# rishikksh20/FastSpeech2

Hardware: NVIDIA H100
Metric: mel-frames/sec (batched inference) (higher is better)
Workload: dtype 3xf16

## Files before the change

fastspeech2_b200/csrc/gemm_tc.cu:

```cuda
#include <stdlib.h>

#include "tc_common.cuh"

namespace fs2 {
namespace {
using namespace tc;

constexpr int BM = 128;
constexpr int BK = 32;
constexpr int A_BYTES = BM * BK * 4;
constexpr int THREADS = 384;
constexpr int RING_BUDGET = 227 * 1024 - 1024  - 256 ;

struct TcParams {
  int L, tiles_per_utt;
  int m_tiles, n_tiles;
  int B, full, gn, upt, full_tiles;
  int K, taps, pad;
  const float* bias; const float* resid; int ldr; int act;
  float* out; int ldo;
  float a_inv; const float* w_inv;
  __half* outp; __half* outp_lo; int ldo_p;
  float* vt_out; __half* vtp; __half* vtp_lo; int vt_col0, vt_dk, vt_heads, vt_lpad, vt_L;
  const int64_t* lens;
};

template <int BN, bool PRECISE, bool HALF = false>
struct Cfg {
  static constexpr int B_BYTES = BN * BK * 4;
  static constexpr int STAGE_BYTES = (PRECISE ? 2 : 1) * (A_BYTES + B_BYTES);
  static_assert(!PRECISE || HALF, "the error-compensated family is 3xF16");
  static constexpr int STAGES = (RING_BUDGET / STAGE_BYTES) > 8 ? 8 : (RING_BUDGET / STAGE_BYTES);
  static constexpr size_t SMEM = (size_t)STAGES * STAGE_BYTES + 1024 + 256;
  static constexpr int BKE = HALF ? 2 * BK : BK;
  static constexpr int A_LO = A_BYTES;
  static constexpr int B_HI = PRECISE ? 2 * A_BYTES : A_BYTES;
  static constexpr int B_LO = B_HI + B_BYTES;
  static constexpr uint32_t TX_BYTES = (PRECISE ? 2 : 1) * (A_BYTES + B_BYTES);
  static_assert(BN % 16 == 0 && BN >= 16 && BN <= 128, "tile width: sums of wgmma N = 128 / 64 / 16");
  static_assert(B_BYTES % 1024 == 0, "B stage must keep 1024-byte alignment");
  static_assert(STAGES >= 2, "resources");
};

template <int BN, bool HALF, int C0 = 0>
__device__ __forceinline__ void mma_tile(float* d, uint64_t a, uint64_t b, uint32_t acc) {
  if constexpr (BN - C0 >= 128) {
    if constexpr (HALF) wgmma_f16_n128(d + C0 / 2, a, b + (C0 * 128 >> 4), acc); else wgmma_tf32_n128(d + C0 / 2, a, b + (C0 * 128 >> 4), acc);
    mma_tile<BN, HALF, C0 + 128>(d, a, b, acc);
  } else if constexpr (BN - C0 >= 64) {
    if constexpr (HALF) wgmma_f16_n64(d + C0 / 2, a, b + (C0 * 128 >> 4), acc); else wgmma_tf32_n64(d + C0 / 2, a, b + (C0 * 128 >> 4), acc);
    mma_tile<BN, HALF, C0 + 64>(d, a, b, acc);
  } else if constexpr (BN - C0 >= 16) {
    if constexpr (HALF) wgmma_f16_n16(d + C0 / 2, a, b + (C0 * 128 >> 4), acc); else wgmma_tf32_n16(d + C0 / 2, a, b + (C0 * 128 >> 4), acc);
    mma_tile<BN, HALF, C0 + 16>(d, a, b, acc);
  }
}

template <int BN, bool PRECISE, bool HALF>
__global__ void __launch_bounds__(THREADS, 1)
tap_gemm_tc_kernel(const __grid_constant__ CUtensorMap tmap_a, const __grid_constant__ CUtensorMap tmap_b,
                   const __grid_constant__ CUtensorMap tmap_b_lo, const __grid_constant__ CUtensorMap tmap_a16, TcParams p) {
  using C = Cfg<BN, PRECISE, HALF>;
  extern __shared__ uint8_t smem_raw[];
  uint8_t* tiles = smem_raw + ((1024u - (smem_u32(smem_raw) & 1023u)) & 1023u);
  uint64_t* full_bar = reinterpret_cast<uint64_t*>(tiles + (size_t)C::STAGES * C::STAGE_BYTES);
  uint64_t* empty_bar = full_bar + C::STAGES;

  const int warp = uniform_warp_idx(), lane = threadIdx.x & 31;
  const int kchunks = (p.K + C::BKE - 1) / C::BKE;
  const int steps = p.taps * kchunks;
  const int total_tiles = p.m_tiles * p.n_tiles;

  if (threadIdx.x == 0) {
    for (int s = 0; s < C::STAGES; ++s) { mbar_init(&full_bar[s], 1); mbar_init(&empty_bar[s], 8); }
    asm volatile("fence.mbarrier_init.release.cluster;" ::: "memory");
  }
  __syncthreads();
  pdl_wait();

  auto tile_coords = [&](int tile, int& n0, int& b, int& t0, int& packed) -> bool {
    const int mt = tile / p.n_tiles;
    n0 = (tile - mt * p.n_tiles) * BN;
    packed = -1;
    if (p.tiles_per_utt == 0) { b = 0; t0 = mt * BM; }
    else if (mt < p.full_tiles) { b = mt / p.full; t0 = (mt - b * p.full) * BM; }
    else { packed = mt - p.full_tiles; b = packed * p.upt; t0 = p.full * BM; }
    return packed < 0 && p.lens != nullptr && t0 >= p.lens[b];
  };

  if (warp == 0) {
    const uint32_t tiles_addr = smem_u32(tiles), full_addr = smem_u32(full_bar);
    int n = 0;
    for (int tile = blockIdx.x; tile < total_tiles; tile += gridDim.x) {
      int n0, b, t0, packed;
      if (tile_coords(tile, n0, b, t0, packed)) continue;
      int j = 0, kc = 0;
      for (int s = 0; s < steps; ++s, ++n) {
        const int slot = n % C::STAGES, round = n / C::STAGES;
        const int k0 = kc * C::BKE, row = t0 + j - p.pad;
        const uint32_t st = tiles_addr + (uint32_t)slot * C::STAGE_BYTES, fb = full_addr + (uint32_t)slot * 8u;
        pin_before(st, fb, k0, row);
        mbar_wait(&empty_bar[slot], (round & 1) ^ 1);
        mbar_expect_tx_elect(fb, C::TX_BYTES);
        if (packed < 0) {
          tma_load_3d_elect(st, &tmap_a, fb, k0, row, b);
          if (PRECISE) tma_load_3d_elect(st + C::A_LO, &tmap_a, fb, k0, row, b + p.B);
        } else {
          for (int g = 0; g < 8; ++g) {
            const int u = g / p.gn, gi = g - u * p.gn;
            const bool real = u < p.upt && b + u < p.B;
            const int oob = PRECISE ? 2 * p.B : p.B;
            tma_load_3d_elect(st + g * (16 * 128), &tmap_a16, fb, k0, row + gi * 16, real ? b + u : oob);
            if (PRECISE) tma_load_3d_elect(st + C::A_LO + g * (16 * 128), &tmap_a16, fb, k0, row + gi * 16, real ? b + u + p.B : oob);
          }
        }
        tma_load_3d_elect(st + C::B_HI, &tmap_b, fb, k0, n0, j);
        if (PRECISE) tma_load_3d_elect(st + C::B_LO, &tmap_b_lo, fb, k0, n0, j);
        if (++kc == kchunks) { kc = 0; ++j; }
      }
    }
  } else if (warp >= 4) {
    const int cg = (warp >> 2) - 1, wq = warp & 3;
    const int r_lo = 64 * cg + 16 * wq + (lane >> 2);
    const int act = p.act, ldr = p.ldr, ldo = p.ldo;
    const float* __restrict__ resid = p.resid; float* __restrict__ out = p.out;
    const bool has_res = resid != nullptr;
    const float oscale = p.a_inv * (p.w_inv ? __ldg(p.w_inv) : 1.0f);
    float d[BN / 2];
    int n = 0;
    for (int tile = blockIdx.x; tile < total_tiles; tile += gridDim.x) {
      int n0, b, t0, packed;
      const int tile_steps = tile_coords(tile, n0, b, t0, packed) ? 0 : steps;
      long m[2]; bool row_ok[2], row_zero[2];
#pragma unroll
      for (int h = 0; h < 2; ++h) {
        const int row = r_lo + 8 * h;
        int bb = b, t = t0 + row;
        bool ok = t < p.L;
        if (packed >= 0) {
          const int g = row >> 4, u = g / p.gn, gi = g - u * p.gn;
          bb += u;
          t = t0 + gi * 16 + (row & 15);
          ok = u < p.upt && bb < p.B && t < p.L;
        }
        m[h] = (long)bb * p.L + t; row_ok[h] = ok;
        row_zero[h] = ok && p.lens != nullptr && t >= p.lens[bb];
        if (has_res && ok) prefetch_l2(resid + m[h] * ldr + n0);
      }
      int prev = -1;
      for (int s = 0; s < tile_steps; ++s, ++n) {
        const int slot = n % C::STAGES, round = n / C::STAGES;
        const uint32_t base = smem_u32(tiles + (size_t)slot * C::STAGE_BYTES);
        const uint64_t a_hi = make_sw128_kmajor_desc(base + cg * (A_BYTES / 2)), b_hi = make_sw128_kmajor_desc(base + C::B_HI);
        const uint64_t a_lo = make_sw128_kmajor_desc(base + C::A_LO + cg * (A_BYTES / 2)), b_lo = make_sw128_kmajor_desc(base + C::B_LO);
        mbar_wait(&full_bar[slot], round & 1);
        wgmma_fence();
#pragma unroll
        for (int k = 0; k < 4; ++k) {
          if (PRECISE) {
            mma_tile<BN, true>(d, a_lo + 2 * k, b_hi + 2 * k, (s | k) != 0);
            mma_tile<BN, true>(d, a_hi + 2 * k, b_lo + 2 * k, 1);
            mma_tile<BN, true>(d, a_hi + 2 * k, b_hi + 2 * k, 1);
          } else {
            mma_tile<BN, HALF>(d, a_hi + 2 * k, b_hi + 2 * k, (s | k) != 0);
          }
        }
        wgmma_commit();
        wgmma_wait<1>();
        pin_regs<BN / 2>(d);
        if (prev >= 0) { __syncwarp(); if (lane == 0) mbar_arrive(&empty_bar[prev]); }
        prev = slot;
      }
      wgmma_wait<0>();
      pin_regs<BN / 2>(d);
      if (prev >= 0) { __syncwarp(); if (lane == 0) mbar_arrive(&empty_bar[prev]); }
      if (tile_steps == 0) {
#pragma unroll
        for (int i = 0; i < BN / 2; ++i) d[i] = 0.f;
      }

      const bool to_vt = (p.vt_out != nullptr || p.vtp != nullptr) && n0 >= p.vt_col0;
#pragma unroll
      for (int h = 0; h < 2; ++h) {
        if (!row_ok[h] || (to_vt && row_zero[h])) continue;
        const long mm = m[h];
#pragma unroll
        for (int jj = 0; jj < BN / 8; ++jj) {
          const int c = 8 * jj + 2 * (lane & 3), col = n0 + c;
          float v0 = d[4 * jj + 2 * h], v1 = d[4 * jj + 2 * h + 1];
          const float b0 = p.bias ? __ldg(p.bias + col) : 0.f, b1 = p.bias ? __ldg(p.bias + col + 1) : 0.f;
          v0 = fmaf(v0, oscale, b0); v1 = fmaf(v1, oscale, b1);
          if (to_vt) {
            const long ub = mm / p.vt_L; const int ut = (int)(mm - ub * p.vt_L);
            const int rel = col - p.vt_col0, hh = rel / p.vt_dk, d0 = rel - hh * p.vt_dk;
            const long o = ((ub * p.vt_heads + hh) * p.vt_dk + d0) * (long)p.vt_lpad + ut;
            if (p.vt_out != nullptr) {
              p.vt_out[o] = v0; p.vt_out[o + p.vt_lpad] = v1;
            } else {
              uint32_t hi, lo;
              split_pair(v0, v1, hi, lo);
              const __half2 h2 = *reinterpret_cast<const __half2*>(&hi), l2 = *reinterpret_cast<const __half2*>(&lo);
              p.vtp[o] = __low2half(h2); p.vtp[o + p.vt_lpad] = __high2half(h2);
              if (p.vtp_lo != nullptr) { p.vtp_lo[o] = __low2half(l2); p.vtp_lo[o + p.vt_lpad] = __high2half(l2); }
            }
            continue;
          }
          if (act == ACT_RELU) { v0 = fmaxf(v0, 0.f); v1 = fmaxf(v1, 0.f); }
          else if (act == ACT_TANH) { v0 = tanhf(v0); v1 = tanhf(v1); }
          if (has_res) {
            const float2 r = __ldg(reinterpret_cast<const float2*>(resid + mm * ldr + col));
            v0 += r.x; v1 += r.y;
          }
          if (row_zero[h]) { v0 = 0.f; v1 = 0.f; }
          if (HALF && p.outp != nullptr) {
            const long off = mm * p.ldo_p + col;
            if (p.outp_lo != nullptr) {
              uint32_t hi, lo;
              split_pair(v0, v1, hi, lo);
              *reinterpret_cast<uint32_t*>(p.outp + off) = hi;
              *reinterpret_cast<uint32_t*>(p.outp_lo + off) = lo;
            } else {
              *reinterpret_cast<uint32_t*>(p.outp + off) = hi_pair(v0, v1);
            }
          }
          if (out != nullptr) *reinterpret_cast<float2*>(out + mm * ldo + col) = make_float2(v0, v1);
        }
      }
    }
  }
  pdl_trigger();
}

__global__ void split_rows_f16_kernel(const float* __restrict__ x, int ldx, long rows, int K, __half* __restrict__ S) {
  pdl_trigger(); pdl_wait();
  const int kq = K >> 2;
  const long quads = rows * kq;
  __half* __restrict__ lo_plane = S + rows * K;
  for (long i = (long)blockIdx.x * blockDim.x + threadIdx.x; i < quads; i += (long)gridDim.x * blockDim.x) {
    const long r = i / kq;
    const int c = (int)(i - r * kq) * 4;
    const float4 v = *reinterpret_cast<const float4*>(x + r * ldx + c);
    uint2 hv, lv;
    split_pair(v.x, v.y, hv.x, lv.x);
    split_pair(v.z, v.w, hv.y, lv.y);
    *reinterpret_cast<uint2*>(S + r * K + c) = hv;
    *reinterpret_cast<uint2*>(lo_plane + r * K + c) = lv;
  }
}

template <int BN, bool PRECISE, bool HALF = false>
int launch(const TapGemm& g, cudaStream_t st) {
  using C = Cfg<BN, PRECISE, HALF>;
  static unsigned long long configured = 0;
  int rc;
  if ((rc = ensure_smem_attr(tap_gemm_tc_kernel<BN, PRECISE, HALF>, C::SMEM, &configured))) return rc;
  TcParams p;
  p.K = g.K; p.taps = g.taps; p.pad = (g.taps - 1) / 2;
  p.bias = g.bias; p.resid = g.resid; p.ldr = g.ldr; p.act = g.act; p.out = g.out; p.ldo = g.ldo;
  const long rows = (long)g.B * g.L;
  p.a_inv = HALF ? g.a_inv : 1.0f; p.w_inv = HALF ? g.w_inv : nullptr;
  p.outp = HALF ? g.outp : nullptr; p.ldo_p = g.ldo_p;
  p.outp_lo = (HALF && g.outp && g.outp_lo) ? g.outp + rows * g.ldo_p : nullptr;
  p.vt_out = HALF ? nullptr : g.vt_out; p.vtp = HALF ? g.vtp : nullptr;
  p.vtp_lo = (HALF && g.vtp && g.outp_lo) ? g.vtp + (long)g.B * g.vt_heads * g.vt_dk * g.vt_lpad : nullptr;
  p.vt_col0 = g.vt_col0; p.vt_dk = g.vt_dk; p.vt_heads = g.vt_heads; p.vt_lpad = g.vt_lpad; p.vt_L = g.L;
  p.lens = g.lens;
  CUtensorMap ma, mb, mb_lo, ma16;
  const int esz = HALF ? 2 : 4;
  constexpr int planes = HALF && PRECISE ? 2 : 1;
  const void* xa = HALF ? (const void*)g.xp : (const void*)g.x;
  const uint64_t row_bytes = HALF ? (uint64_t)g.K * 2 : (uint64_t)g.ldx * 4;
  if (g.taps == 1 && g.lens == nullptr) {
    const uint64_t M = (uint64_t)g.B * g.L;
    p.L = (int)M; p.tiles_per_utt = 0;
    p.m_tiles = (int)((M + BM - 1) / BM);
    p.B = 1; p.full = 0; p.gn = 1; p.upt = 1; p.full_tiles = 0;
    if ((rc = make_map(&ma, xa, g.K, M, planes, row_bytes, row_bytes * M, BM, HALF))) return rc;
    ma16 = ma;
  } else {
    p.L = g.L; p.tiles_per_utt = (g.L + BM - 1) / BM;
    p.B = g.B; p.full = g.L / BM;
    int tail = g.L % BM;
    p.gn = tail ? (tail + 15) / 16 : 1;
    p.upt = tail ? 8 / p.gn : 1;
    if (tail && p.upt == 1) { p.full += 1; tail = 0; p.gn = 1; }
    p.full_tiles = p.full * g.B;
    p.m_tiles = p.full_tiles + (tail ? (g.B + p.upt - 1) / p.upt : 0);
    if ((rc = make_map(&ma, xa, g.K, g.L, (uint64_t)g.B * planes, row_bytes, row_bytes * g.L, BM, HALF))) return rc;
    if ((rc = make_map(&ma16, xa, g.K, g.L, (uint64_t)g.B * planes, row_bytes, row_bytes * g.L, 16, HALF))) return rc;
  }
  p.n_tiles = g.N / BN;
  const void* w_hi = HALF ? (const void*)g.w_hi : (const void*)g.w;
  if ((rc = make_map(&mb, w_hi, g.K, g.N, g.taps, (uint64_t)g.K * esz, (uint64_t)g.K * esz * g.N, BN, HALF))) return rc;
  if ((rc = make_map(&mb_lo, PRECISE ? (const void*)g.w_lo : w_hi, g.K, g.N, g.taps, (uint64_t)g.K * esz, (uint64_t)g.K * esz * g.N, BN, HALF))) return rc;
  const int total = p.m_tiles * p.n_tiles;
  const int grid = total < sm_count_current() ? total : sm_count_current();
  FS2_CUDA_CHECK(launch_pdl(tap_gemm_tc_kernel<BN, PRECISE, HALF>, dim3(grid), dim3(THREADS), C::SMEM, st, ma, mb, mb_lo, ma16, p));
  FS2_LAUNCH_CHECK();
  return FS2_OK;
}

int tile_width(int N) { return N % 128 == 0 ? 128 : N % 80 == 0 ? 80 : N % 64 == 0 ? 64 : N % 32 == 0 ? 32 : 16; }

template <bool PRECISE, bool HALF>
int launch_any(const TapGemm& g, cudaStream_t st) {
  switch (tile_width(g.N)) {
    case 128: return launch<128, PRECISE, HALF>(g, st);
    case 80: return launch<80, PRECISE, HALF>(g, st);
    case 64: return launch<64, PRECISE, HALF>(g, st);
    case 32: return launch<32, PRECISE, HALF>(g, st);
    default: return launch<16, PRECISE, HALF>(g, st);
  }
}

int check_output(const TapGemm& g, const char* who) {
  FS2_REQUIRE((g.taps & 1) == 1, "%s: taps must be odd", who);
  FS2_REQUIRE(g.N % 16 == 0, "%s: N (%d) must be a multiple of 16", who, g.N);
  FS2_REQUIRE(!g.resid || g.ldr % 4 == 0, "%s: row strides must be 16-byte multiples", who);
  FS2_REQUIRE(!g.out || (g.ldo % 8 == 0 && (reinterpret_cast<uintptr_t>(g.out) & 31) == 0), "%s: output rows must be 32-byte aligned", who);
  return FS2_OK;
}
int check_common(const TapGemm& g, const char* who) {
  FS2_REQUIRE(g.K % 4 == 0, "%s: K (%d) must be a multiple of 4", who, g.K);
  FS2_REQUIRE(g.ldx % 4 == 0, "%s: row strides must be 16-byte multiples", who);
  FS2_REQUIRE((reinterpret_cast<uintptr_t>(g.x) & 15) == 0 && (reinterpret_cast<uintptr_t>(g.w) & 15) == 0 && g.out != nullptr,
              "%s: operands must be 16-byte aligned", who);
  return check_output(g, who);
}

}

int tap_gemm_tf32(const TapGemm& g, cudaStream_t st) {
  int rc = check_common(g, "tap_gemm_tf32");
  if (rc) return rc;
  if ((long)g.B * g.L == 0) return FS2_OK;
  return launch_any<false, false>(g, st);
}

int tap_gemm_planes(const TapGemm& g, cudaStream_t st) {
  const char* who = g.precise ? "tap_gemm_planes(3xF16)" : "tap_gemm_planes(f16)";
  FS2_REQUIRE(g.xp && g.w_hi && (!g.precise || g.w_lo) && (g.out || g.outp || g.vtp), "%s: operand planes / an output missing", who);
  FS2_REQUIRE(g.K % 8 == 0, "%s: K (%d) must be a multiple of 8 (16-byte plane rows)", who, g.K);
  FS2_REQUIRE((reinterpret_cast<uintptr_t>(g.xp) & 15) == 0 && (reinterpret_cast<uintptr_t>(g.w_hi) & 15) == 0, "%s: operands must be 16-byte aligned", who);
  FS2_REQUIRE(!g.outp || (g.ldo_p % 16 == 0 && (reinterpret_cast<uintptr_t>(g.outp) & 31) == 0 && (((long)g.B * g.L * g.ldo_p) % 16) == 0),
              "%s: output plane rows must be 32-byte aligned", who);
  {
    const int bn = tile_width(g.N);
    FS2_REQUIRE(!g.vtp || (g.vt_lpad % 8 == 0 && g.N % bn == 0 && g.vt_col0 % bn == 0 && g.vt_dk % 32 == 0),
                "%s: transposed V planes need a 16-byte row pitch and tile-aligned thirds", who);
  }
  int rc = check_output(g, who);
  if (rc) return rc;
  if ((long)g.B * g.L == 0) return FS2_OK;
  return g.precise ? launch_any<true, true>(g, st) : launch_any<false, true>(g, st);
}

int split_rows(const float* x, int ldx, long rows, int K, __half* planes, cudaStream_t st) {
  if (rows == 0) return FS2_OK;
  FS2_REQUIRE(K % 4 == 0 && ldx % 4 == 0, "split_rows: K and the row stride must be multiples of 4");
  const long quads = rows * (K / 4);
  long blocks = (quads + 255) / 256;
  FS2_CUDA_CHECK(launch_pdl(split_rows_f16_kernel, dim3((unsigned)(blocks > 132 * 16 ? 132 * 16 : blocks)), dim3(256), 0, st, x, ldx, rows, K, planes));
  FS2_LAUNCH_CHECK();
  return FS2_OK;
}

namespace {
__global__ void split_f16_kernel(const float* __restrict__ src, __half* __restrict__ hi, __half* __restrict__ lo, long n,
                                 const float* __restrict__ scale) {
  const float s = scale ? __ldg(scale) : 1.0f;
  for (long i = (long)blockIdx.x * blockDim.x + threadIdx.x; i < n; i += (long)gridDim.x * blockDim.x) {
    const float x = fminf(fmaxf(src[i] * s, -65504.f), 65504.f);
    const __half h = __float2half_rn(x);
    hi[i] = h; lo[i] = __float2half_rn(x - __half2float(h));
  }
}
__global__ void weight_scale_kernel(const float* __restrict__ w, long n, float* __restrict__ scale, float* __restrict__ inv) {
  __shared__ float red[32];
  float m = 0.f;
  for (long i = threadIdx.x; i < n; i += blockDim.x) m = fmaxf(m, fabsf(w[i]));
  m = warp_max(m);
  if ((threadIdx.x & 31) == 0) red[threadIdx.x >> 5] = m;
  __syncthreads();
  if (threadIdx.x < 32) {
    m = threadIdx.x < (blockDim.x >> 5) ? red[threadIdx.x] : 0.f;
    m = warp_max(m);
    if (threadIdx.x == 0) {
      int k = 0;
      if (m > 0.f && isfinite(m)) {
        int e;
        frexpf(m, &e);
        k = 14 - e;
        k = k > 60 ? 60 : (k < -60 ? -60 : k);
      }
      scale[0] = ldexpf(1.0f, k); inv[0] = ldexpf(1.0f, -k);
    }
  }
}
}

namespace {
__global__ void planes_to_rows_kernel(const __half* __restrict__ planes, long n, float* __restrict__ out) {
  for (long i = (long)blockIdx.x * blockDim.x + threadIdx.x; i < n; i += (long)gridDim.x * blockDim.x)
    out[i] = (__half2float(planes[i]) + __half2float(planes[n + i])) * kPlaneInv;
}
}

int planes_to_rows(const __half* planes, long n, float* out, cudaStream_t st) {
  if (n == 0) return FS2_OK;
  long blocks = (n + 255) / 256;
  planes_to_rows_kernel<<<(int)(blocks > 1184 ? 1184 : blocks), 256, 0, st>>>(planes, n, out);
  FS2_LAUNCH_CHECK();
  return FS2_OK;
}

int split_f16(const float* src, __half* hi, __half* lo, long n, const float* scale, cudaStream_t st) {
  if (n == 0) return FS2_OK;
  long blocks = (n + 255) / 256;
  split_f16_kernel<<<(int)(blocks > 1184 ? 1184 : blocks), 256, 0, st>>>(src, hi, lo, n, scale);
  FS2_LAUNCH_CHECK();
  return FS2_OK;
}

int weight_scale(const float* w, long n, float* scale, float* inv, cudaStream_t st) {
  weight_scale_kernel<<<1, 1024, 0, st>>>(w, n, scale, inv);
  FS2_LAUNCH_CHECK();
  return FS2_OK;
}

}
```

Baseline: 2.897 million.

## Ping-pong consumer warpgroups over whole tiles with register reallocation

```diff
diff --git a/fastspeech2_b200/csrc/gemm_tc.cu b/fastspeech2_b200/csrc/gemm_tc.cu
--- a/fastspeech2_b200/csrc/gemm_tc.cu
+++ b/fastspeech2_b200/csrc/gemm_tc.cu
@@ -10,6 +10,7 @@
 constexpr int BK = 32;
 constexpr int A_BYTES = BM * BK * 4;
 constexpr int THREADS = 384;
+constexpr int PRODUCER_REGS = 40, CONSUMER_REGS = 232;
 constexpr int RING_BUDGET = 227 * 1024 - 1024  - 256 ;
 
 struct TcParams {
@@ -71,8 +72,11 @@
   const int steps = p.taps * kchunks;
   const int total_tiles = p.m_tiles * p.n_tiles;
 
+  uint64_t* order_bar = empty_bar + C::STAGES;
+
   if (threadIdx.x == 0) {
-    for (int s = 0; s < C::STAGES; ++s) { mbar_init(&full_bar[s], 1); mbar_init(&empty_bar[s], 8); }
+    for (int s = 0; s < C::STAGES; ++s) { mbar_init(&full_bar[s], 1); mbar_init(&empty_bar[s], 4); }
+    mbar_init(&order_bar[0], 4); mbar_init(&order_bar[1], 4);
     asm volatile("fence.mbarrier_init.release.cluster;" ::: "memory");
   }
   __syncthreads();
@@ -88,7 +92,9 @@
     return packed < 0 && p.lens != nullptr && t0 >= p.lens[b];
   };
 
-  if (warp == 0) {
+  if (warp < 4) {
+    setmaxnreg_dec<PRODUCER_REGS>();
+    if (warp != 0) { pdl_trigger(); return; }
     const uint32_t tiles_addr = smem_u32(tiles), full_addr = smem_u32(full_bar);
     int n = 0;
     for (int tile = blockIdx.x; tile < total_tiles; tile += gridDim.x) {
@@ -119,22 +125,25 @@
         if (++kc == kchunks) { kc = 0; ++j; }
       }
     }
-  } else if (warp >= 4) {
+  } else {
+    setmaxnreg_inc<CONSUMER_REGS>();
     const int cg = (warp >> 2) - 1, wq = warp & 3;
-    const int r_lo = 64 * cg + 16 * wq + (lane >> 2);
+    const int r_lo = 16 * wq + (lane >> 2);
     const int act = p.act, ldr = p.ldr, ldo = p.ldo;
     const float* __restrict__ resid = p.resid; float* __restrict__ out = p.out;
     const bool has_res = resid != nullptr;
     const float oscale = p.a_inv * (p.w_inv ? __ldg(p.w_inv) : 1.0f);
-    float d[BN / 2];
+    float d[BN];
     int n = 0;
-    for (int tile = blockIdx.x; tile < total_tiles; tile += gridDim.x) {
+    int k = 0;
+    for (int tile = blockIdx.x; tile < total_tiles; tile += gridDim.x, ++k) {
       int n0, b, t0, packed;
       const int tile_steps = tile_coords(tile, n0, b, t0, packed) ? 0 : steps;
-      long m[2]; bool row_ok[2], row_zero[2];
-#pragma unroll
-      for (int h = 0; h < 2; ++h) {
-        const int row = r_lo + 8 * h;
+      if ((k & 1) != cg) { n += tile_steps; continue; }
+      long m[4]; bool row_ok[4], row_zero[4];
+#pragma unroll
+      for (int i = 0; i < 4; ++i) {
+        const int row = 64 * (i >> 1) + r_lo + 8 * (i & 1);
         int bb = b, t = t0 + row;
         bool ok = t < p.L;
         if (packed >= 0) {
@@ -143,57 +152,81 @@
           t = t0 + gi * 16 + (row & 15);
           ok = u < p.upt && bb < p.B && t < p.L;
         }
-        m[h] = (long)bb * p.L + t; row_ok[h] = ok;
-        row_zero[h] = ok && p.lens != nullptr && t >= p.lens[bb];
-        if (has_res && ok) prefetch_l2(resid + m[h] * ldr + n0);
-      }
+        m[i] = (long)bb * p.L + t; row_ok[i] = ok;
+        row_zero[i] = ok && p.lens != nullptr && t >= p.lens[bb];
+        if (has_res && ok) prefetch_l2(resid + m[i] * ldr + n0);
+      }
+      if (k > 0) mbar_wait(&order_bar[cg], ((k - 1) >> 1) & 1);
       int prev = -1;
       for (int s = 0; s < tile_steps; ++s, ++n) {
         const int slot = n % C::STAGES, round = n / C::STAGES;
         const uint32_t base = smem_u32(tiles + (size_t)slot * C::STAGE_BYTES);
-        const uint64_t a_hi = make_sw128_kmajor_desc(base + cg * (A_BYTES / 2)), b_hi = make_sw128_kmajor_desc(base + C::B_HI);
-        const uint64_t a_lo = make_sw128_kmajor_desc(base + C::A_LO + cg * (A_BYTES / 2)), b_lo = make_sw128_kmajor_desc(base + C::B_LO);
+        const uint64_t a_hi = make_sw128_kmajor_desc(base), b_hi = make_sw128_kmajor_desc(base + C::B_HI);
+        const uint64_t a_lo = make_sw128_kmajor_desc(base + C::A_LO), b_lo = make_sw128_kmajor_desc(base + C::B_LO);
+        constexpr uint64_t HALF_A = (A_BYTES / 2) >> 4;
         mbar_wait(&full_bar[slot], round & 1);
         wgmma_fence();
 #pragma unroll
-        for (int k = 0; k < 4; ++k) {
-          if (PRECISE) {
-            mma_tile<BN, true>(d, a_lo + 2 * k, b_hi + 2 * k, (s | k) != 0);
-            mma_tile<BN, true>(d, a_hi + 2 * k, b_lo + 2 * k, 1);
-            mma_tile<BN, true>(d, a_hi + 2 * k, b_hi + 2 * k, 1);
-          } else {
-            mma_tile<BN, HALF>(d, a_hi + 2 * k, b_hi + 2 * k, (s | k) != 0);
+        for (int kk = 0; kk < 4; ++kk) {
+#pragma unroll
+          for (int hf = 0; hf < 2; ++hf) {
+            float* dh = d + hf * (BN / 2);
+            if (PRECISE) {
+              mma_tile<BN, true>(dh, a_lo + hf * HALF_A + 2 * kk, b_hi + 2 * kk, (s | kk) != 0);
+              mma_tile<BN, true>(dh, a_hi + hf * HALF_A + 2 * kk, b_lo + 2 * kk, 1);
+              mma_tile<BN, true>(dh, a_hi + hf * HALF_A + 2 * kk, b_hi + 2 * kk, 1);
+            } else {
+              mma_tile<BN, HALF>(dh, a_hi + hf * HALF_A + 2 * kk, b_hi + 2 * kk, (s | kk) != 0);
+            }
           }
         }
         wgmma_commit();
         wgmma_wait<1>();
-        pin_regs<BN / 2>(d);
+        pin_regs<BN>(d);
         if (prev >= 0) { __syncwarp(); if (lane == 0) mbar_arrive(&empty_bar[prev]); }
         prev = slot;
       }
+      __syncwarp();
+      if (lane == 0) mbar_arrive(&order_bar[cg ^ 1]);
       wgmma_wait<0>();
-      pin_regs<BN / 2>(d);
+      pin_regs<BN>(d);
       if (prev >= 0) { __syncwarp(); if (lane == 0) mbar_arrive(&empty_bar[prev]); }
       if (tile_steps == 0) {
 #pragma unroll
-        for (int i = 0; i < BN / 2; ++i) d[i] = 0.f;
+        for (int i = 0; i < BN; ++i) d[i] = 0.f;
       }
 
       const bool to_vt = (p.vt_out != nullptr || p.vtp != nullptr) && n0 >= p.vt_col0;
 #pragma unroll
-      for (int h = 0; h < 2; ++h) {
-        if (!row_ok[h] || (to_vt && row_zero[h])) continue;
-        const long mm = m[h];
+      for (int i = 0; i < 4; ++i) {
+        if (!row_ok[i] || (to_vt && row_zero[i])) continue;
+        const long mm = m[i];
+        float* dr = d + (i >> 1) * (BN / 2) + 2 * (i & 1);
 #pragma unroll
         for (int jj = 0; jj < BN / 8; ++jj) {
-          const int c = 8 * jj + 2 * (lane & 3), col = n0 + c;
-          float v0 = d[4 * jj + 2 * h], v1 = d[4 * jj + 2 * h + 1];
+          const int col = n0 + 8 * jj + 2 * (lane & 3);
+          float v0 = dr[4 * jj], v1 = dr[4 * jj + 1];
           const float b0 = p.bias ? __ldg(p.bias + col) : 0.f, b1 = p.bias ? __ldg(p.bias + col + 1) : 0.f;
           v0 = fmaf(v0, oscale, b0); v1 = fmaf(v1, oscale, b1);
-          if (to_vt) {
-            const long ub = mm / p.vt_L; const int ut = (int)(mm - ub * p.vt_L);
-            const int rel = col - p.vt_col0, hh = rel / p.vt_dk, d0 = rel - hh * p.vt_dk;
-            const long o = ((ub * p.vt_heads + hh) * p.vt_dk + d0) * (long)p.vt_lpad + ut;
+          if (!to_vt) {
+            if (act == ACT_RELU) { v0 = fmaxf(v0, 0.f); v1 = fmaxf(v1, 0.f); }
+            else if (act == ACT_TANH) { v0 = tanhf(v0); v1 = tanhf(v1); }
+            if (has_res) {
+              const float2 r = __ldg(reinterpret_cast<const float2*>(resid + mm * ldr + col));
+              v0 += r.x; v1 += r.y;
+            }
+            if (row_zero[i]) { v0 = 0.f; v1 = 0.f; }
+          }
+          dr[4 * jj] = v0; dr[4 * jj + 1] = v1;
+        }
+        if (to_vt) {
+          const long ub = mm / p.vt_L;
+          const long orow = ub * p.vt_heads * p.vt_dk * (long)p.vt_lpad + (mm - ub * p.vt_L);
+#pragma unroll
+          for (int jj = 0; jj < BN / 8; ++jj) {
+            const int col = n0 + 8 * jj + 2 * (lane & 3);
+            const float v0 = dr[4 * jj], v1 = dr[4 * jj + 1];
+            const long o = orow + (long)(col - p.vt_col0) * p.vt_lpad;
             if (p.vt_out != nullptr) {
               p.vt_out[o] = v0; p.vt_out[o + p.vt_lpad] = v1;
             } else {
@@ -203,15 +236,13 @@
               p.vtp[o] = __low2half(h2); p.vtp[o + p.vt_lpad] = __high2half(h2);
               if (p.vtp_lo != nullptr) { p.vtp_lo[o] = __low2half(l2); p.vtp_lo[o + p.vt_lpad] = __high2half(l2); }
             }
-            continue;
           }
-          if (act == ACT_RELU) { v0 = fmaxf(v0, 0.f); v1 = fmaxf(v1, 0.f); }
-          else if (act == ACT_TANH) { v0 = tanhf(v0); v1 = tanhf(v1); }
-          if (has_res) {
-            const float2 r = __ldg(reinterpret_cast<const float2*>(resid + mm * ldr + col));
-            v0 += r.x; v1 += r.y;
-          }
-          if (row_zero[h]) { v0 = 0.f; v1 = 0.f; }
+          continue;
+        }
+#pragma unroll
+        for (int jj = 0; jj < BN / 8; ++jj) {
+          const int col = n0 + 8 * jj + 2 * (lane & 3);
+          const float v0 = dr[4 * jj], v1 = dr[4 * jj + 1];
           if (HALF && p.outp != nullptr) {
             const long off = mm * p.ldo_p + col;
             if (p.outp_lo != nullptr) {
```

Result: faster. 3.000 million (median of 6 runs) (+3.6%).
